# carolinebear/pytorch_end2end_speech_recognition

Measured on AMD Instinct MI355X. Metric: training frames/sec, higher is better.
Workload: dtype bf16; 1 GPU; librispeech100h_char_ctc_blstm5x512; batch_per_gpu=32, global_batch=32, max_frames=1000, feat_dim=80, vocab=29, parallelism=dp1

## Files before the change

### include/asr_hip.h

```cpp
#ifndef ASR_HIP_H_
#define ASR_HIP_H_

#include <stddef.h>
#include <stdint.h>

#ifdef __cplusplus
extern "C" {
#endif

#define ASR_OK 0
#define ASR_ERR_ARG (-1)
#define ASR_ERR_WORKSPACE (-2)
#define ASR_ERR_HIP (-3)
#define ASR_ERR_UNSUPPORTED (-4)

#define ASR_DT_F32 0
#define ASR_DT_BF16 1

const char* asr_version(void);
const char* asr_last_error(void);
int asr_arch_is_gfx950(void);

int asr_stream_create_cu_masked(int cu_begin, int cu_count, void** stream_out);
int asr_stream_destroy(void* stream);

size_t asr_ctc_workspace_bytes(int T, int B, int V, int max_label_len);
int asr_ctc_forward(const float* acts, long long stride_t, long long stride_b, int T, int B,
                    int V, const int32_t* labels_flat, const int32_t* label_lens,
                    const int32_t* act_lens, int max_label_len, int blank, int zero_infinity,
                    float* costs, float* loss_out, float loss_scale, void* workspace,
                    size_t ws_bytes, void* stream);
int asr_ctc_forward_lse(const float* acts, long long stride_t, long long stride_b, int T, int B,
                        int V, const float* lse_part, int nslab, const int32_t* labels_flat,
                        const int32_t* label_lens, const int32_t* act_lens, int max_label_len,
                        int blank, int zero_infinity, float* costs, float* loss_out,
                        float loss_scale, void* workspace, size_t ws_bytes, void* stream);
int asr_ctc_backward(const float* acts, long long stride_t, long long stride_b, int T, int B,
                     int V, const int32_t* labels_flat, const int32_t* label_lens,
                     const int32_t* act_lens, int max_label_len, int blank,
                     const float* grad_scale, float scale, float* grads, long long gstride_t,
                     long long gstride_b, const void* workspace, size_t ws_bytes, void* stream);
int asr_ctc_backward_bf16(const float* acts, long long stride_t, long long stride_b, int T, int B,
                          int V, const int32_t* labels_flat, const int32_t* label_lens,
                          const int32_t* act_lens, int max_label_len, int blank,
                          const float* grad_scale, float scale, uint16_t* grads,
                          long long gstride_t, long long gstride_b, int gld,
                          const void* workspace, size_t ws_bytes, void* stream);
size_t asr_ctc_bias_workspace_bytes(int T, int B, int V, int gld);
int asr_ctc_backward_bf16_db(const float* acts, long long stride_t, long long stride_b, int T,
                             int B, int V, const int32_t* labels_flat, const int32_t* label_lens,
                             const int32_t* act_lens, int max_label_len, int blank,
                             const float* grad_scale, float scale, uint16_t* grads,
                             long long gstride_t, long long gstride_b, int gld,
                             const void* workspace, size_t ws_bytes, float* dbias, void* bias_ws,
                             size_t bias_ws_bytes, void* stream);
int asr_ctc_fwd_bwd(const float* acts, long long stride_t, long long stride_b, int T, int B,
                    int V, const int32_t* labels_flat, const int32_t* label_lens,
                    const int32_t* act_lens, int max_label_len, int blank, int zero_infinity,
                    float* costs, float* grads, void* workspace, size_t ws_bytes, void* stream);

int asr_ctc_last_path(int* out2);
int asr_ctc_last_lattice_waves(void);
int asr_gemm_last_family(void);

typedef struct {
  long long stride_b;
  long long stride_t;
  int rows_per_b;
  int t_mul;
  int t_add;
  int t_limit;
  const int32_t* perm;
} asr_rowmap_t;

typedef struct {
  const void* ptr;
  int dtype;
  int trans;
  asr_rowmap_t map;
  long long bytes;
  int tap_group;
  int tap_pitch;
  int tap_sign;
} asr_operand_t;

typedef struct {
  asr_operand_t a;
  asr_operand_t b;
  float* c;
  asr_rowmap_t c_map;
  const float* bias;
  const float* bias2;
  int M, N, K;
  float alpha, beta;
  int batch;
  long long batch_stride_a, batch_stride_b, batch_stride_c;
  float drop_p;
  unsigned long long drop_seed;
  int c_dtype;
} asr_gemm_t;

typedef struct { int small_tiles, nosplit, n64_kmode; } asr_gemm_opts_t;

int asr_gemm(const asr_gemm_t* problems, int nprob, int compute_dtype, void* stream,
             const asr_gemm_opts_t* opts);

size_t asr_gemm_workspace_bytes(const asr_gemm_t* problems, int nprob,
                                const asr_gemm_opts_t* opts);
int asr_gemm_ws(const asr_gemm_t* problems, int nprob, int compute_dtype, void* workspace,
                size_t ws_bytes, void* stream, const asr_gemm_opts_t* opts);
int asr_gemm_lse_ws(const asr_gemm_t* problem, int compute_dtype, float* lse, void* workspace,
                    size_t ws_bytes, void* stream, const asr_gemm_opts_t* opts);

int asr_lstm_wgrad_gate(void* stream);

size_t asr_colsum_workspace_bytes(int M, int N);
int asr_colsum_accumulate(const float* g, long long ld, int M, int N, float alpha, float* out0,
                          float* out1, void* workspace, size_t ws_bytes, void* stream);
int asr_colsum_accumulate_bf16(const uint16_t* g, long long ld, int M, int N, float alpha,
                               float* out0, float* out1, void* workspace, size_t ws_bytes,
                               void* stream);

typedef struct {
  int ws_prezeroed, bwd_pin_kb, bwd_units;
  const int* dy_flags;
  int dy_c0, dy_epoch;
  unsigned long long* progress;
  int progress_q1, progress_q2;
} asr_lstm_opts_t;
size_t asr_lstm_workspace_bytes(int B, int H, int compute_dtype, int backward);
int asr_lstm_forward(float* gx_act, const void* whh_f, const void* whh_r, int w_dtype,
                     const int32_t* lens, int B, int T, int H, int compute_dtype, float* y,
                     float* cst, uint16_t* ybf, void* workspace, size_t ws_bytes, void* stream,
                     const asr_lstm_opts_t* opts);
int asr_lstm_backward(const float* dy, const void* whh_f, const void* whh_r, int w_dtype,
                      const int32_t* lens, int B, int T, int H, int compute_dtype, float* act_dg,
                      const float* cst, uint16_t* dgbf, void* workspace, size_t ws_bytes,
                      void* stream, const asr_lstm_opts_t* opts);
// ... 453 lines not shown
```

### pytorch_end2end_speech_recognition_amd/_native.py

```python
import ctypes
import os

import torch

_HERE = os.path.dirname(os.path.abspath(__file__))
LIB_PATH = os.environ.get('ASR_LIB_PATH') or os.path.join(_HERE, 'libasr_hip.so')

c_int = ctypes.c_int
c_ll = ctypes.c_longlong
c_float = ctypes.c_float
c_size = ctypes.c_size_t
c_vp = ctypes.c_void_p
c_str = ctypes.c_char_p

ASR_OK = 0
ASR_ERR_UNSUPPORTED = -4
ASR_DT_F32 = 0
ASR_DT_BF16 = 1

SIGNATURES = {
    'asr_version': (c_str, []),
    'asr_last_error': (c_str, []),
    'asr_arch_is_gfx950': (c_int, []),
    'asr_stream_create_cu_masked': (c_int, [c_int, c_int, c_vp]),
    'asr_stream_destroy': (c_int, [c_vp]),
    'asr_ctc_workspace_bytes': (c_size, [c_int, c_int, c_int, c_int]),
    'asr_ctc_forward': (c_int, [c_vp, c_ll, c_ll, c_int, c_int, c_int, c_vp, c_vp, c_vp, c_int,
                                c_int, c_int, c_vp, c_vp, c_float, c_vp, c_size, c_vp]),
    'asr_ctc_forward_lse': (c_int, [c_vp, c_ll, c_ll, c_int, c_int, c_int, c_vp, c_int, c_vp,
                                    c_vp, c_vp, c_int, c_int, c_int, c_vp, c_vp, c_float, c_vp,
                                    c_size, c_vp]),
    'asr_ctc_backward': (c_int, [c_vp, c_ll, c_ll, c_int, c_int, c_int, c_vp, c_vp, c_vp, c_int,
                                 c_int, c_vp, c_float, c_vp, c_ll, c_ll, c_vp, c_size, c_vp]),
    'asr_ctc_backward_bf16': (c_int, [c_vp, c_ll, c_ll, c_int, c_int, c_int, c_vp, c_vp, c_vp,
                                      c_int, c_int, c_vp, c_float, c_vp, c_ll, c_ll, c_int, c_vp,
                                      c_size, c_vp]),
    'asr_ctc_bias_workspace_bytes': (c_size, [c_int, c_int, c_int, c_int]),
    'asr_ctc_backward_bf16_db': (c_int, [c_vp, c_ll, c_ll, c_int, c_int, c_int, c_vp, c_vp, c_vp,
                                         c_int, c_int, c_vp, c_float, c_vp, c_ll, c_ll, c_int, c_vp,
                                         c_size, c_vp, c_vp, c_size, c_vp]),
    'asr_ctc_fwd_bwd': (c_int, [c_vp, c_ll, c_ll, c_int, c_int, c_int, c_vp, c_vp, c_vp, c_int,
                                c_int, c_int, c_vp, c_vp, c_vp, c_size, c_vp]),
    'asr_gemm': (c_int, [c_vp, c_int, c_int, c_vp, c_vp]),
    'asr_gemm_workspace_bytes': (c_size, [c_vp, c_int, c_vp]),
    'asr_gemm_ws': (c_int, [c_vp, c_int, c_int, c_vp, c_size, c_vp, c_vp]),
    'asr_gemm_lse_ws': (c_int, [c_vp, c_int, c_vp, c_vp, c_size, c_vp, c_vp]),
    'asr_lstm_wgrad_gate': (c_int, [c_vp]),
    'asr_colsum_workspace_bytes': (c_size, [c_int, c_int]),
    'asr_colsum_accumulate': (c_int, [c_vp, c_ll, c_int, c_int, c_float, c_vp, c_vp, c_vp, c_size,
                                      c_vp]),
    'asr_colsum_accumulate_bf16': (c_int, [c_vp, c_ll, c_int, c_int, c_float, c_vp, c_vp, c_vp,
                                           c_size, c_vp]),
    'asr_conv3x3_c1_forward_xs': (c_int, [c_vp, c_int, c_int, c_int, c_int, c_int, c_vp, c_vp,
                                          c_vp, c_int, c_vp]),
    'asr_conv3x3_tr_supported': (c_int, [c_int, c_int, c_int]),
    'asr_conv3x3_tr': (c_int, [c_vp, c_ll, c_int, c_int, c_int, c_vp, c_int, c_vp, c_vp, c_int,
                               c_vp]),
    'asr_vgg_zero_halo': (c_int, [c_vp, c_int, c_int, c_int, c_int, c_int, c_vp]),
    'asr_conv3x3_c1_wgrad_workspace_bytes': (c_size, [c_int]),
    'asr_conv3x3_c1_wgrad_xs': (c_int, [c_vp, c_int, c_int, c_int, c_int, c_int, c_vp, c_int, c_vp,
                                        c_vp, c_size, c_vp]),
    'asr_conv3x3_tr_wgrad_workspace_bytes': (c_size, [c_ll, c_int, c_int, c_int]),
    'asr_conv3x3_tr_wgrad': (c_int, [c_vp, c_vp, c_ll, c_int, c_int, c_int, c_vp, c_vp, c_size,
                                     c_vp]),
    'asr_conv3x3_c1_forward': (c_int, [c_vp, c_int, c_int, c_int, c_int, c_int, c_int, c_vp, c_vp,
                                       c_vp, c_vp]),
    'asr_lstm_workspace_bytes': (c_size, [c_int, c_int, c_int, c_int]),
    'asr_lstm_forward': (c_int, [c_vp, c_vp, c_vp, c_int, c_vp, c_int, c_int, c_int, c_int, c_vp,
                                 c_vp, c_vp, c_vp, c_size, c_vp, c_vp]),
    'asr_lstm_backward': (c_int, [c_vp, c_vp, c_vp, c_int, c_vp, c_int, c_int, c_int, c_int,
                                  c_vp, c_vp, c_vp, c_vp, c_size, c_vp, c_vp]),
    'asr_lstm_backward_db': (c_int, [c_vp, c_vp, c_vp, c_int, c_vp, c_int, c_int, c_int, c_int,
                                     c_vp, c_vp, c_vp, c_vp, c_vp, c_vp, c_size, c_vp, c_vp]),
    'asr_lstm_backward_dgbf': (c_int, [c_vp, c_vp, c_vp, c_int, c_vp, c_int, c_int, c_int, c_int,
                                       c_vp, c_vp, c_vp, c_vp, c_vp, c_vp, c_size, c_vp, c_vp]),
    'asr_lstm_forward_x': (c_int, [c_vp, c_int, c_vp, c_vp, c_vp, c_vp, c_vp, c_vp, c_int, c_int,
                                   c_int, c_vp, c_vp, c_vp, c_vp, c_vp, c_size, c_vp, c_vp]),
    'asr_lstm_forward_x_ok': (c_int, [c_int, c_int, c_int]),
    'asr_lstm_forward_xh': (c_int, [c_vp, c_int, c_vp, c_vp, c_vp, c_vp, c_vp, c_vp, c_int, c_int,
                                    c_int, c_vp, c_vp, c_vp, c_vp, c_vp, c_size, c_vp, c_vp]),
    'asr_lstm_forward_xh_drop': (c_int, [c_vp, c_int, c_vp, c_vp, c_vp, c_vp, c_vp, c_vp, c_int,
                                         c_int, c_int, c_vp, c_vp, c_vp, c_vp, c_vp, c_float,
                                         ctypes.c_ulonglong, c_vp, c_size, c_vp, c_vp]),
    'asr_lstm_backward_dgbf_h': (c_int, [c_vp, c_vp, c_vp, c_int, c_vp, c_int, c_int, c_int, c_int,
                                         c_vp, c_vp, c_vp, c_vp, c_vp, c_vp, c_size, c_vp, c_vp]),
    'asr_diag_lds_spin': (c_int, [c_int, c_int, c_vp, c_vp]),
    'asr_diag_hold_cus': (c_int, [c_int, c_int, c_int, c_vp]),
    'asr_lstm_unpack_act_h': (c_int, [c_vp, c_int, c_int, c_int, c_vp, c_vp]),
    'asr_gru_workspace_bytes': (c_size, [c_int, c_int]),
    'asr_gru_forward': (c_int, [c_vp, c_vp, c_vp, c_vp, c_int, c_int, c_int, c_vp, c_vp, c_vp]),
    'asr_gru_backward': (c_int, [c_vp, c_vp, c_vp, c_int, c_int, c_int, c_vp, c_vp, c_vp, c_vp,
                                 c_vp, c_size, c_vp]),
    'asr_gru_cell_forward': (c_int, [c_vp, c_vp, c_vp, c_int, c_int, c_vp, c_vp, c_vp]),
    'asr_gru_cell_backward': (c_int, [c_vp, c_vp, c_vp, c_vp, c_int, c_int, c_vp, c_vp, c_vp,
                                      c_vp]),
    'asr_grad_sqnorm_workspace_bytes': (c_size, []),
    'asr_grad_sqnorm': (c_int, [c_vp, c_ll, c_vp, c_vp, c_size, c_vp]),
    'asr_optim_step': (c_int, [c_int, c_vp, c_vp, c_vp, c_vp, c_ll, c_float, c_float, c_float,
                               c_float, c_float, c_ll, c_float, c_float, c_vp, c_float, c_vp,
                               c_vp]),
    'asr_optim_step_guarded': (c_int, [c_int, c_vp, c_vp, c_vp, c_vp, c_ll, c_float, c_float,
                                       c_float, c_float, c_float, c_ll, c_float, c_float, c_vp,
                                       c_float, c_vp, c_vp, c_vp]),
    'asr_dropout': (c_int, [c_vp, c_vp, c_ll, c_float, ctypes.c_ulonglong, c_vp]),
    'asr_embedding_forward': (c_int, [c_vp, c_vp, c_int, c_int, c_int, c_int, c_vp, c_vp]),
    'asr_embedding_backward': (c_int, [c_vp, c_vp, c_int, c_int, c_int, c_int, c_int, c_vp,
                                       c_vp]),
    'asr_embedding_backward_csr': (c_int, [c_vp, c_vp, c_vp, c_int, c_int, c_int, c_int, c_vp,
                                           c_vp]),
    'asr_tanh_forward': (c_int, [c_vp, c_vp, c_ll, c_vp]),
    'asr_tanh_backward': (c_int, [c_vp, c_vp, c_vp, c_ll, c_vp]),
    'asr_add_tanh_forward': (c_int, [c_vp, c_vp, c_vp, c_ll, c_vp]),
    'asr_add_forward': (c_int, [c_vp, c_vp, c_vp, c_ll, c_vp]),
    'asr_convert_rows_bf16': None,
    'asr_convert_rows_bf16_dropout': None,
    'asr_ctc_best_path': (c_int, [c_vp, c_ll, c_ll, c_int, c_int, c_int, c_vp, c_int, c_vp, c_vp,
                                  c_vp]),
    'asr_row_argmax': (c_int, [c_vp, c_int, c_int, c_vp, c_vp]),
    'asr_ctc_beam_ws_bytes': (c_size, [c_int, c_int, c_int, c_int]),
    'asr_ctc_beam_search': (c_int, [c_vp, c_ll, c_ll, c_int, c_int, c_int, c_vp, c_int, c_int,
                                    c_int, c_vp, c_size, c_vp, c_vp, c_vp, c_vp]),
    'asr_ctc_beam_rows': (c_int, [c_vp, c_ll, c_ll, c_int, c_int, c_int, c_vp, c_int, c_int, c_int,
                                  c_vp, c_size, c_vp]),
# ... 291 lines not shown
```

### pytorch_end2end_speech_recognition_amd/csrc/ctc.hip

```cpp
#include "common.h"
#include "prof.h"

namespace asr {
namespace {

constexpr int kMaxK = 16;

struct CtcWs {
  float* lse;
  float* emit;
  float* alpha;
  float* beta;
  float* logp;
  int32_t* offs;
  int32_t* status;
};

inline size_t align256(size_t x) { return (x + 255) & ~size_t(255); }

inline int pick_k(int max_label_len) {
  int S = 2 * max_label_len + 1;
  int k = 1;
  while (64 * k < S) k <<= 1;
  return k;
}

inline size_t ws_layout(int T, int B, int max_label_len, CtcWs* ws, char* base) {
  const int Spad = 64 * pick_k(max_label_len);
  size_t off = 0;
  auto take = [&](size_t bytes) { size_t o = off; off = align256(off + bytes); return base + o; };
  char* p;
  p = take(sizeof(float) * (size_t)B * T);                 if (ws) ws->lse = (float*)p;
  p = take(sizeof(float) * (size_t)B * T * Spad);          if (ws) ws->emit = (float*)p;
  p = take(sizeof(float) * (size_t)B * T * Spad);          if (ws) ws->alpha = (float*)p;
  p = take(sizeof(float) * (size_t)B * T * Spad);          if (ws) ws->beta = (float*)p;
  p = take(sizeof(float) * (size_t)B);                     if (ws) ws->logp = (float*)p;
  p = take(sizeof(int32_t) * (size_t)B);                   if (ws) ws->offs = (int32_t*)p;
  p = take(sizeof(int32_t) * 4);                           if (ws) ws->status = (int32_t*)p;
  return off;
}

__global__ void ctc_prep(const int32_t* __restrict__ label_lens, const int32_t* __restrict__ labels,
                         int B, int V, int blank, int max_label_len, int32_t* __restrict__ offs,
                         int32_t* __restrict__ status) {
  if (threadIdx.x == 0) {
    int acc = 0, bad = 0;
    for (int b = 0; b < B; ++b) {
      offs[b] = acc;
      int L = label_lens[b];
      if (L < 0 || L > max_label_len) bad |= 1;
      acc += L < 0 ? 0 : L;
    }
    status[0] = bad;
    status[1] = acc;
  }
  __syncthreads();
  int total = status[1];
  for (int i = threadIdx.x; i < total; i += blockDim.x) {
    int v = labels[i];
    if (v < 0 || v >= V || v == blank) atomicOr(&status[0], 2);
  }
}

__device__ __forceinline__ void lds_barrier() {
  asm volatile("s_waitcnt lgkmcnt(0)\n\ts_barrier" ::: "memory");
}

constexpr float kLog2e = 1.4426950408889634f;
constexpr float kLn2 = 0.6931471805599453f;
__device__ __forceinline__ float ex2(float x) { return __builtin_amdgcn_exp2f(x); }
__device__ __forceinline__ float lg2(float x) { return __builtin_amdgcn_logf(x); }

__device__ __forceinline__ void lse_acc4(float& m, float& s, float4 v) {
  const float mx = fmaxf(fmaxf(v.x, v.y), fmaxf(v.z, v.w));
  if (mx > m) { s *= __expf(m - mx); m = mx; }
  s += __expf(v.x - m) + __expf(v.y - m) + __expf(v.z - m) + __expf(v.w - m);
}
__device__ __forceinline__ void lse_acc1(float& m, float& s, float x) {
  if (x > m) { s *= __expf(m - x); m = x; }
  s += __expf(x - m);
}

__device__ __forceinline__ int head_elems(const float* p) {
// ... 982 lines not shown
  extern __shared__ __attribute__((aligned(16))) float lds_n[];
  const int lane = threadIdx.x & 63, wave = threadIdx.x >> 6;
  float* occ = lds_n + wave * V;
  const int n8 = gld >> 3;
  const float scale = (grad_scale ? grad_scale[0] : 1.0f) * scale_mul;
  float acc[NCH][8];
#pragma unroll
  for (int j = 0; j < NCH; ++j)
#pragma unroll
    for (int e = 0; e < 8; ++e) acc[j][e] = 0.f;
  for (int r = wave; r < rpb; r += NW) {
    const long long lin = (long long)blockIdx.x * rpb + r;
    if (lin >= nrows) break;
    const long long row = rev ? nrows - 1 - lin : lin;
    const int b = (int)(row / T), t = (int)(row % T);
    uint16_t* g = grads + (long long)t * gst + (long long)b * gsb;
    const float* x = acts + (long long)t * st + (long long)b * sb;
    const int Tb = act_lens[b];
    const float lp = logp[b];
    if (t >= Tb || lp == neg_inf()) {
      for (int i = lane; i < n8; i += 64) reinterpret_cast<uint4*>(g)[i] = make_uint4(0u, 0u, 0u, 0u);
      continue;
    }
    float xv[NCH][8];
#pragma unroll
    for (int j = 0; j < NCH; ++j)
#pragma unroll
      for (int e = 0; e < 8; ++e) {
        const int c = 8 * (lane + 64 * j) + e;
        xv[j][e] = c < V ? x[c] : 0.f;
      }
    const float z = lse[row];
    const int L = min(label_lens[b], (Spad - 1) / 2);
    const int S = 2 * L + 1;
    const int32_t* lab = labels + offs[b];
    const float* al = alpha + row * Spad;
    const float* bt = beta + row * Spad;
    const float* em = emit + row * Spad;
    for (int v = lane; v < V; v += 64) occ[v] = 0.f;
    __builtin_amdgcn_fence(__ATOMIC_RELEASE, "wavefront");
    __builtin_amdgcn_wave_barrier();
    for (int s_ = lane; s_ < S; s_ += 64) {
      int c = (s_ & 1) ? lab[s_ >> 1] : blank;
      c = c < 0 ? 0 : (c >= V ? V - 1 : c);
      atomicAdd(&occ[c], ex2(al[s_] + bt[s_] - em[s_] - lp));
    }
    __builtin_amdgcn_fence(__ATOMIC_ACQ_REL, "wavefront");
    __builtin_amdgcn_wave_barrier();
#pragma unroll
    for (int j = 0; j < NCH; ++j) {
      const int k = lane + 64 * j;
      if (k >= n8) continue;
      unsigned w[4];
#pragma unroll
      for (int q = 0; q < 4; ++q) {
        const int c = 8 * k + 2 * q;
        const float lo = c < V ? (__expf(xv[j][2 * q] - z) - occ[c]) * scale : 0.f;
        const float hi = c + 1 < V ? (__expf(xv[j][2 * q + 1] - z) - occ[c + 1]) * scale : 0.f;
        acc[j][2 * q] += lo;
        acc[j][2 * q + 1] += hi;
        w[q] = (c < V ? (unsigned)f2bf(lo) : 0u) | ((c + 1 < V ? (unsigned)f2bf(hi) : 0u) << 16);
      }
      reinterpret_cast<uint4*>(g)[k] = make_uint4(w[0], w[1], w[2], w[3]);
    }
    __builtin_amdgcn_fence(__ATOMIC_ACQ_REL, "wavefront");
    __builtin_amdgcn_wave_barrier();
  }
  if (!colpart) return;
  float* wp = lds_n + NW * V;
#pragma unroll
  for (int j = 0; j < NCH; ++j) {
    const int k = lane + 64 * j;
    if (k >= n8) continue;
#pragma unroll
    for (int e = 0; e < 8; ++e) wp[wave * gld + 8 * k + e] = acc[j][e];
  }
  __syncthreads();
  float* o = colpart + (long long)blockIdx.x * gld;
  for (int c = threadIdx.x; c < gld; c += 64 * NW) {
    float v = wp[c];
#pragma unroll
    for (int w = 1; w < NW; ++w) v += wp[w * gld + c];
    o[c] = v;
  }
}

template <int NCH>
__global__ void __launch_bounds__(256) ctc_grad_bf16_pipe(
    const float* __restrict__ acts, long long st, long long sb, int T, int V,
    const int32_t* __restrict__ labels, const int32_t* __restrict__ label_lens,
    const int32_t* __restrict__ act_lens, const int32_t* __restrict__ offs, int blank, int Spad,
    const float* __restrict__ lse, const float* __restrict__ emit,
    const float* __restrict__ alpha, const float* __restrict__ beta,
    const float* __restrict__ logp, const float* __restrict__ grad_scale, float scale_mul,
    uint16_t* __restrict__ grads, long long gst, long long gsb, int gld, int rev,
    int acts_bytes, float* __restrict__ colpart, int rpb, long long nrows) {
  extern __shared__ __attribute__((aligned(16))) float occ[];
  float* corr = occ + Spad;
  int* clsT = (int*)(occ + Spad + V);
  __shared__ int s_b;
  const int tid = threadIdx.x, nth = blockDim.x;
  const int n8 = gld >> 3;
  const float scale = (grad_scale ? grad_scale[0] : 1.0f) * scale_mul;
  const __amdgpu_buffer_rsrc_t rs =
      __builtin_amdgcn_make_buffer_rsrc((void*)acts, 0, acts_bytes, 0x00020000);
  float acc[NCH > 0 ? NCH : 1][8];
#pragma unroll
  for (int j = 0; j < (NCH > 0 ? NCH : 1); ++j)
#pragma unroll
    for (int e = 0; e < 8; ++e) acc[j][e] = 0.f;
  for (int v = tid; v < V; v += nth) corr[v] = 0.f;
  if (tid == 0) s_b = -1;
  struct Row { long long row; int b, t, Tb, L; float lp, z; float sv[4]; };
  auto fetch = [&](int r, Row& h) {
    const long long lin = (long long)blockIdx.x * rpb + r;
    h.row = rev ? nrows - 1 - lin : lin;
    h.b = (int)(h.row / T);
    h.t = (int)(h.row % T);
    h.Tb = act_lens[h.b];
    h.lp = logp[h.b];
    h.z = lse[h.row];
    h.L = label_lens[h.b];
    const long long so = h.row * Spad;
#pragma unroll
    for (int q = 0; q < 4; ++q) {
      const int s_ = tid + q * nth;
      h.sv[q] = s_ < Spad ? alpha[so + s_] + beta[so + s_] - emit[so + s_] : 0.f;
    }
  };
  const int nr = (int)min((long long)rpb, nrows - (long long)blockIdx.x * rpb);
  Row cur;
  if (nr > 0) fetch(0, cur);
  for (int r = 0; r < nr; ++r) {
    const int b = cur.b, t = cur.t;
    uint16_t* g = grads + (long long)t * gst + (long long)b * gsb;
    const bool live = t < cur.Tb && cur.lp != neg_inf();
    const int L = min(cur.L, (Spad - 1) / 2);
    const int S = 2 * L + 1;
    __syncthreads();
    if (live && s_b != b) {
      const int32_t* lab = labels + offs[b];
      for (int s_ = tid; s_ < S; s_ += nth) {
        int c = (s_ & 1) ? lab[s_ >> 1] : blank;
        clsT[s_] = c < 0 ? 0 : (c >= V ? V - 1 : c);
      }
    }
    if (live) {
#pragma unroll
      for (int q = 0; q < 4; ++q) {
        const int s_ = tid + q * nth;
        if (s_ < S) occ[s_] = ex2(cur.sv[q] - cur.lp);
      }
    }
    __syncthreads();
    if (tid == 0 && live) s_b = b;
    int rep_c[4] = {-1, -1, -1, -1};
    if (live) {
#pragma unroll
      for (int q4 = 0; q4 < 4; ++q4) {
        const int s_ = tid + q4 * nth;
        if (s_ >= S) continue;
        const int c = clsT[s_];
        bool first;
        if ((s_ & 1) == 0) {
          first = s_ == 0;
        } else {
// ... 606 lines not shown
#define ASR_CTC_GS(NC)                                                                           \
  hipLaunchKernelGGL((ctc_grad_bf16_stream<NC>), dim3((unsigned)nblk), dim3(512), lds2, s, acts, \
                     stride_t, stride_b, T, V, labels_flat, label_lens, act_lens, ws.offs, blank, \
                     Spad, ws.lse, ws.emit, ws.alpha, ws.beta, ws.logp, grad_scale, scale, grads, \
                     gstride_t, gstride_b, gld, rev, abytes, colpart, rpb, rows)
    switch (nchs) {
      case 1: ASR_CTC_GS(1); break;
      case 2: ASR_CTC_GS(2); break;
      default: ASR_CTC_GS(3); break;
    }
#undef ASR_CTC_GS
  } else
#define ASR_CTC_GP(NC)                                                                           \
  hipLaunchKernelGGL((ctc_grad_bf16_pipe<NC>), dim3((unsigned)nblk), dim3(threads), lds, s, acts, \
                     stride_t, stride_b, T, V, labels_flat, label_lens, act_lens, ws.offs, blank, \
                     Spad, ws.lse, ws.emit, ws.alpha, ws.beta, ws.logp, grad_scale, scale, grads, \
                     gstride_t, gstride_b, gld, rev, abytes, colpart, rpb, rows)
  if (pipe) {
    g_ctc_last_path[1] = 3;
    switch (nch) {
      case 1: ASR_CTC_GP(1); break;
      case 2: ASR_CTC_GP(2); break;
      case 4: ASR_CTC_GP(4); break;
      case 5: ASR_CTC_GP(5); break;
      default: ASR_CTC_GP(8); break;
    }
  } else if (table) {
    g_ctc_last_path[1] = 1;
    if (nch) ASR_CTC_G16A(true, 1, false);
    else ASR_CTC_G16A(true, 0, false);
  } else {
    g_ctc_last_path[1] = 1;
    switch (nch) {
      case 0: ASR_CTC_G16(false, 0); break;
      case 1: ASR_CTC_G16(false, 1); break;
      case 2: ASR_CTC_G16(false, 2); break;
      case 4: ASR_CTC_G16(false, 4); break;
      case 5: ASR_CTC_G16(false, 5); break;
      default: ASR_CTC_G16(false, 8); break;
    }
  }
#undef ASR_CTC_G16A
#undef ASR_CTC_GP
#undef ASR_CTC_G16
  ASR_LAUNCH_CHECK();
  prof_end_launch(ASR_PROF_CTC_GRAD, pslot, s);
  if (dbias) {
    const size_t part = ((size_t)nblk * gld * sizeof(float) + 255) & ~(size_t)255;
    rc = asr_colsum_accumulate(colpart, gld, nblk, V, 1.0f, dbias, nullptr, (char*)bws + part,
                               bws_bytes - part, stream);
    if (rc) return rc;
  }
  return ASR_OK;
}

extern "C" int asr_ctc_backward_bf16(const float* acts, long long stride_t, long long stride_b,
                                     int T, int B, int V, const int32_t* labels_flat,
                                     const int32_t* label_lens, const int32_t* act_lens,
                                     int max_label_len, int blank, const float* grad_scale,
                                     float scale, uint16_t* grads, long long gstride_t,
                                     long long gstride_b, int gld, const void* workspace,
                                     size_t ws_bytes, void* stream) {
  return ctc_backward_bf16_impl(acts, stride_t, stride_b, T, B, V, labels_flat, label_lens,
                                act_lens, max_label_len, blank, grad_scale, scale, grads,
                                gstride_t, gstride_b, gld, workspace, ws_bytes, nullptr, nullptr, 0,
                                stream);
}

extern "C" int asr_ctc_backward_bf16_db(const float* acts, long long stride_t, long long stride_b,
                                        int T, int B, int V, const int32_t* labels_flat,
                                        const int32_t* label_lens, const int32_t* act_lens,
                                        int max_label_len, int blank, const float* grad_scale,
                                        float scale, uint16_t* grads, long long gstride_t,
                                        long long gstride_b, int gld, const void* workspace,
                                        size_t ws_bytes, float* dbias, void* bias_ws,
                                        size_t bias_ws_bytes, void* stream) {
  ASR_REQUIRE(dbias, ASR_ERR_ARG, "ctc_bf16_db: dbias is null");
  return ctc_backward_bf16_impl(acts, stride_t, stride_b, T, B, V, labels_flat, label_lens,
                                act_lens, max_label_len, blank, grad_scale, scale, grads,
                                gstride_t, gstride_b, gld, workspace, ws_bytes, dbias, bias_ws,
                                bias_ws_bytes, stream);
}

extern "C" int asr_ctc_fwd_bwd(const float* acts, long long stride_t, long long stride_b, int T,
                               int B, int V, const int32_t* labels_flat,
                               const int32_t* label_lens, const int32_t* act_lens,
                               int max_label_len, int blank, int zero_infinity, float* costs,
                               float* grads, void* workspace, size_t ws_bytes, void* stream) {
  int rc = asr_ctc_forward(acts, stride_t, stride_b, T, B, V, labels_flat, label_lens, act_lens,
                           max_label_len, blank, zero_infinity, costs, nullptr, 1.f, workspace,
                           ws_bytes, stream);
  if (rc || !grads) return rc;
  return asr_ctc_backward(acts, stride_t, stride_b, T, B, V, labels_flat, label_lens, act_lens,
                          max_label_len, blank, nullptr, 1.f, grads, stride_t, stride_b, workspace,
                          ws_bytes, stream);
}
```

### pytorch_end2end_speech_recognition_amd/native_ops.py

```python
import collections
import ctypes
import os
import weakref

import numpy as np
import torch

from . import _native as N

F32 = N.ASR_DT_F32
BF16 = N.ASR_DT_BF16

_compute = {'dtype': F32}


def set_compute_dtype(name):
    if name not in ('fp32', 'bf16'):
        raise ValueError('compute dtype must be fp32 or bf16')
    _compute['dtype'] = BF16 if name == 'bf16' else F32


def compute_dtype():
    return _compute['dtype']

# ... 406 lines not shown
        ctx.beside = _beside_plan[0]
        return y

    @staticmethod
    def backward(ctx, dy):
        xo, wo = ctx.saved_tensors
        bias, stage, xshape, weight = ctx.meta
        dy = dy.contiguous()
        Nout = weight.shape[0]
        M = dy.numel() // Nout
        if M == 0:
            return torch.zeros(xshape, dtype=torch.float32, device=dy.device), None, None, None
        Np = wo.shape[0] if stage else Nout
        dyo = _staged(dy, M, Nout, Np) if stage else dy
        if ctx.beside is not None:
            dx = _linear_backward(xo, wo, bias, stage, xshape, weight, ctx.drop, dyo,
                                  ctx.needs_input_grad[0], dy_bias=dy, wgrad=False)
            gb = (grad_buffer(weight),) + ((grad_buffer(bias),) if bias is not None else ())
            wgrad = lambda go: _linear_wgrad(xo, wo, bias, stage, xshape, weight, dyo,
                                             dy_bias=dy, gemm_opts=go)
            if not _wgrad_beside(dy.device, ctx.beside, wgrad, (xo, wo, dyo, dy), gb):
                wgrad(None)
            return dx, None, None, None
        dx = _linear_backward(xo, wo, bias, stage, xshape, weight, ctx.drop, dyo,
                              ctx.needs_input_grad[0], dy_bias=dy)
        return dx, None, None, None


def _ctc_forward(logits, st, sb, T, B, V, lse, labels_flat, label_lens, act_lens, max_label_len,
                 blank, zero_infinity, costs, loss, loss_scale, ws, nbytes):
    common = (N.ptr(labels_flat), N.ptr(label_lens), N.ptr(act_lens), int(max_label_len),
              int(blank), int(bool(zero_infinity)), N.ptr(costs), N.ptr(loss), float(loss_scale),
              N.ptr(ws), nbytes, N.stream_handle(logits.device))
    if lse is not None:
        N.call('asr_ctc_forward_lse', N.ptr(logits), st, sb, T, B, V, N.ptr(lse), lse.shape[0],
               *common)
    else:
        N.call('asr_ctc_forward', N.ptr(logits), st, sb, T, B, V, *common)


class LinearCTCFn(torch.autograd.Function):

    @staticmethod
    def forward(ctx, x, weight, bias, drop, labels_flat, label_lens, act_lens, max_label_len,
                loss_scale, blank, zero_infinity):
        N.require_device(labels_flat, label_lens, act_lens)
        V = weight.shape[0]
        M = x.numel() // x.shape[-1]
        lse = (torch.empty((V + 63) // 64, M, 2, dtype=torch.float32, device=x.device)
               if _ctc_lse_epilogue(V) and M > 0 else None)
        logits, xo, wo, stage = _linear_forward(x, weight, bias, drop, lse=lse,
                                                ld=(V + 3) // 4 * 4 if V > 1024 else V)
        assert stage, 'LinearCTCFn needs a staged (bf16) output layer'
        B, T, V = logits.shape
        nbytes = N.query('asr_ctc_workspace_bytes', T, B, V, max_label_len)
        ws = _ws(nbytes, logits.device)
        costs = torch.empty(B, dtype=torch.float32, device=logits.device)
        loss = torch.empty(1, dtype=torch.float32, device=logits.device)
        _ctc_forward(logits, logits.stride(1), logits.stride(0), T, B, V, lse, labels_flat,
                     label_lens, act_lens, max_label_len, blank, zero_infinity, costs, loss,
                     loss_scale, ws, nbytes)
        ctx.save_for_backward(xo, wo, logits, labels_flat, label_lens, act_lens, ws)
        ctx.meta = (bias, tuple(x.shape), weight, int(max_label_len), int(blank),
                    float(loss_scale), nbytes)
        ctx.from_blstm = _produced_by_blstm(x)
        ctx.drop = drop
        ctx.mark_non_differentiable(costs)
        return loss, costs

    @staticmethod
    def backward(ctx, g_loss, g_costs):
        xo, wo, logits, labels_flat, label_lens, act_lens, ws = ctx.saved_tensors
        bias, xshape, weight, max_label_len, blank, loss_scale, nbytes = ctx.meta
        B, T, V = logits.shape
        Np = wo.shape[0]
        dev = logits.device
        dyo = torch.empty(B * T, Np, dtype=torch.bfloat16, device=dev)
        g = g_loss.contiguous() if g_loss is not None else None
        args = (N.ptr(logits), logits.stride(1), logits.stride(0), T, B, V, N.ptr(labels_flat),
                N.ptr(label_lens),
                N.ptr(act_lens), max_label_len, blank, N.ptr(g),
                loss_scale if g is not None else 0.0, N.ptr(dyo), Np, T * Np, Np, N.ptr(ws), nbytes)
        bws = None
        if bias is not None and V <= 16384 and os.environ.get('ASR_CTC_HEAD_DB', '1') != '0':
            bnb = N.query('asr_ctc_bias_workspace_bytes', T, B, V, Np)
            bws = _ws(bnb, dev)
            N.call('asr_ctc_backward_bf16_db', *args, N.ptr(grad_buffer(bias)), N.ptr(bws), bnb,
                   N.stream_handle(dev))
        else:
            N.call('asr_ctc_backward_bf16', *args, N.stream_handle(dev))
        bias_w = None if bws is not None else bias
        if ctx.from_blstm is not None and os.environ.get('ASR_HEAD_WGRAD_SIDE', '1') != '0':
            dx = _linear_backward(xo, wo, bias_w, True, xshape, weight, ctx.drop, dyo,
                                  ctx.needs_input_grad[0], dy_bias=dyo, wgrad=False)
            gb = (grad_buffer(weight),) + ((grad_buffer(bias),) if bias is not None else ())
            wgrad = lambda go: _linear_wgrad(xo, wo, bias_w, True, xshape, weight, dyo,
                                             dy_bias=dyo, gemm_opts=go)
            if not _wgrad_beside(dev, ctx.from_blstm, wgrad, (xo, wo, dyo), gb):
                wgrad(None)
            return (dx,) + (None,) * 10
        dx = _linear_backward(xo, wo, bias_w, True, xshape, weight, ctx.drop, dyo,
                              ctx.needs_input_grad[0], dy_bias=dyo)
        return (dx,) + (None,) * 10


class LinearCTC32Fn(torch.autograd.Function):

    @staticmethod
    def forward(ctx, x, weight, bias, drop, labels_flat, label_lens, act_lens, max_label_len,
                loss_scale, blank, zero_infinity):
        N.require_device(x, weight, labels_flat, label_lens, act_lens)
        ctx.from_blstm = _produced_by_blstm(x)
        x = x.contiguous()
        B, T, K = x.shape
        V = weight.shape[0]
        Vp = (V + 3) // 4 * 4
        dev = x.device
        if drop is not None:
            xd = torch.empty_like(x)
            N.call('asr_dropout', N.ptr(x), N.ptr(xd), x.numel(), float(drop[0]), int(drop[1]),
                   N.stream_handle(dev))
            x = xd
        logits = torch.empty(B * T, Vp, dtype=torch.float32, device=dev)
        lse = (torch.empty((V + 63) // 64, B * T, 2, dtype=torch.float32, device=dev)
               if _ctc_lse_epilogue(V) and B * T > 0 else None)
        if B * T > 0:
            run_gemm([gemm_problem(operand(x, 0, rowmap(K)), operand(weight, 0, rowmap(K)),
                                   logits, rowmap(Vp), B * T, V, K, bias=bias)], dev, lse=lse)
        nbytes = N.query('asr_ctc_workspace_bytes', T, B, V, max_label_len)
        ws = _ws(nbytes, dev)
        costs = torch.empty(B, dtype=torch.float32, device=dev)
        loss = torch.empty(1, dtype=torch.float32, device=dev)
        _ctc_forward(logits, Vp, T * Vp, T, B, V, lse, labels_flat, label_lens, act_lens,
                     max_label_len, blank, zero_infinity, costs, loss, loss_scale, ws, nbytes)
        ctx.save_for_backward(x, logits, labels_flat, label_lens, act_lens, ws)
        ctx.meta = (bias, weight, B, T, V, Vp, int(max_label_len), int(blank), float(loss_scale),
                    nbytes)
        ctx.drop = drop
        ctx.mark_non_differentiable(costs)
        return loss, costs

    @staticmethod
    def backward(ctx, g_loss, g_costs):
        x, logits, labels_flat, label_lens, act_lens, ws = ctx.saved_tensors
        bias, weight, B, T, V, Vp, max_label_len, blank, loss_scale, nbytes = ctx.meta
        dev = logits.device
        K = x.shape[-1]
        M = B * T
        dl = torch.empty(M, Vp, dtype=torch.float32, device=dev)
        g = g_loss.contiguous() if g_loss is not None else None
        N.call('asr_ctc_backward', N.ptr(logits), Vp, T * Vp, T, B, V, N.ptr(labels_flat),
               N.ptr(label_lens), N.ptr(act_lens), max_label_len, blank, N.ptr(g),
               loss_scale if g is not None else 0.0, N.ptr(dl), Vp, T * Vp, N.ptr(ws), nbytes,
               N.stream_handle(dev))
        dx = None
        if ctx.needs_input_grad[0]:
            dx = torch.empty(B, T, K, dtype=torch.float32, device=dev)
            if M > 0:
                run_gemm([gemm_problem(operand(dl, 0, rowmap(Vp)), operand(weight, 1, rowmap(K)),
                                       dx, rowmap(K), M, K, V, drop=ctx.drop)], dev)

        def wgrad(gemm_opts):
            if M > 0:
                run_gemm([gemm_problem(operand(dl, 1, rowmap(Vp)), operand(x, 1, rowmap(K)),
                                       grad_buffer(weight), rowmap(K), V, K, M, beta=1.0)], dev,
                         opts=gemm_opts)
            if bias is not None:
                colsum_accumulate(dl[:, :V], grad_buffer(bias))
        gb = (grad_buffer(weight),) + ((grad_buffer(bias),) if bias is not None else ())
        if not (ctx.from_blstm is not None and os.environ.get('ASR_HEAD_WGRAD_SIDE', '1') != '0'
                and _wgrad_beside(dev, ctx.from_blstm, wgrad, (x, dl), gb)):
            wgrad(None)
        return (dx,) + (None,) * 10


def _produced_by_blstm(t, depth=4):
    frontier = [t.grad_fn] if t.grad_fn is not None else []
    for _ in range(depth):
        nxt = []
        for fn in frontier:
            if fn is None:
                continue
            if type(fn).__name__.startswith('BLSTMLayerFn'):
                return getattr(fn, 'bh', None)
            nxt.extend(f for f, _ in getattr(fn, 'next_functions', ()))
        frontier = nxt
# ... 2365 lines not shown
```

Baseline: 1.760 million frames/s.

## Fuse CTC head gradient with output-projection dgrad GEMM via MFMA

Adds a CTC backward kernel that computes the bf16 logit gradients and, in the same pass, multiplies each 16-row tile by the projection weight with MFMA to produce the input gradient (with dropout applied) directly. The Python autograd path uses it when V<=256 and the shapes fit, and skips the separate dx GEMM. This removes a separate GEMM launch and a re-read of the logit-gradient buffer. In exchange, weights are held in registers, LDS use grows, and the dx GEMM now runs on a narrow 16-row tile that may use MFMA less efficiently than a tuned GEMM.

```diff
diff --git a/include/asr_hip.h b/include/asr_hip.h
--- a/include/asr_hip.h
+++ b/include/asr_hip.h
@@ -54,6 +54,15 @@
                              long long gstride_t, long long gstride_b, int gld,
                              const void* workspace, size_t ws_bytes, float* dbias, void* bias_ws,
                              size_t bias_ws_bytes, void* stream);
+int asr_ctc_backward_bf16_dx_ok(int T, int B, int V, int gld, int K);
+int asr_ctc_backward_bf16_dx(const float* acts, long long stride_t, long long stride_b, int T,
+                             int B, int V, const int32_t* labels_flat, const int32_t* label_lens,
+                             const int32_t* act_lens, int max_label_len, int blank,
+                             const float* grad_scale, float scale, uint16_t* grads,
+                             long long gstride_t, long long gstride_b, int gld,
+                             const void* workspace, size_t ws_bytes, float* dbias, void* bias_ws,
+                             size_t bias_ws_bytes, int fuse_dx, const uint16_t* wo, int K,
+                             float* dx, float drop_p, unsigned long long drop_seed, void* stream);
 int asr_ctc_fwd_bwd(const float* acts, long long stride_t, long long stride_b, int T, int B,
                     int V, const int32_t* labels_flat, const int32_t* label_lens,
                     const int32_t* act_lens, int max_label_len, int blank, int zero_infinity,
diff --git a/pytorch_end2end_speech_recognition_amd/_native.py b/pytorch_end2end_speech_recognition_amd/_native.py
--- a/pytorch_end2end_speech_recognition_amd/_native.py
+++ b/pytorch_end2end_speech_recognition_amd/_native.py
@@ -39,6 +39,11 @@
     'asr_ctc_backward_bf16_db': (c_int, [c_vp, c_ll, c_ll, c_int, c_int, c_int, c_vp, c_vp, c_vp,
                                          c_int, c_int, c_vp, c_float, c_vp, c_ll, c_ll, c_int, c_vp,
                                          c_size, c_vp, c_vp, c_size, c_vp]),
+    'asr_ctc_backward_bf16_dx_ok': (c_int, [c_int, c_int, c_int, c_int, c_int]),
+    'asr_ctc_backward_bf16_dx': (c_int, [c_vp, c_ll, c_ll, c_int, c_int, c_int, c_vp, c_vp, c_vp,
+                                         c_int, c_int, c_vp, c_float, c_vp, c_ll, c_ll, c_int, c_vp,
+                                         c_size, c_vp, c_vp, c_size, c_int, c_vp, c_int, c_vp,
+                                         c_float, ctypes.c_ulonglong, c_vp]),
     'asr_ctc_fwd_bwd': (c_int, [c_vp, c_ll, c_ll, c_int, c_int, c_int, c_vp, c_vp, c_vp, c_int,
                                 c_int, c_int, c_vp, c_vp, c_vp, c_size, c_vp]),
     'asr_gemm': (c_int, [c_vp, c_int, c_int, c_vp, c_vp]),
diff --git a/pytorch_end2end_speech_recognition_amd/csrc/ctc.hip b/pytorch_end2end_speech_recognition_amd/csrc/ctc.hip
--- a/pytorch_end2end_speech_recognition_amd/csrc/ctc.hip
+++ b/pytorch_end2end_speech_recognition_amd/csrc/ctc.hip
@@ -1,4 +1,5 @@
 #include "common.h"
+#include "mfma.h"
 #include "prof.h"
 
 namespace asr {
@@ -1147,6 +1148,159 @@
 #pragma unroll
     for (int w = 1; w < NW; ++w) v += wp[w * gld + c];
     o[c] = v;
+  }
+}
+
+template <int TPW, int KS>
+__global__ void __launch_bounds__(512) ctc_grad_dx_narrow(
+    const float* __restrict__ acts, long long st, long long sb, int T, int V,
+    const int32_t* __restrict__ labels, const int32_t* __restrict__ label_lens,
+    const int32_t* __restrict__ act_lens, const int32_t* __restrict__ offs, int blank, int Spad,
+    const float* __restrict__ lse, const float* __restrict__ emit,
+    const float* __restrict__ alpha, const float* __restrict__ beta,
+    const float* __restrict__ logp, const float* __restrict__ grad_scale, float scale_mul,
+    uint16_t* __restrict__ grads, long long gst, long long gsb, int gld, int rev,
+    float* __restrict__ colpart, int rpb, int nsub, long long nblk, long long nrows,
+    const uint16_t* __restrict__ wo, int K, float* __restrict__ dx, float drop_p,
+    unsigned long long drop_seed) {
+  constexpr int NW = 8;
+  extern __shared__ __attribute__((aligned(16))) float lds_x[];
+  const int lane = threadIdx.x & 63;
+  const int wave = __builtin_amdgcn_readfirstlane(threadIdx.x >> 6);
+  float* occ = lds_x + wave * V;
+  float* rowval = lds_x + NW * V;
+  const int apitch = gld + 8;
+  uint16_t* atile = reinterpret_cast<uint16_t*>(rowval + (colpart ? 2 * 16 * gld : 0));
+  const int n8 = gld >> 3;
+  const int RW = nsub * rpb;
+  const long long nruns = (nrows + RW - 1) / RW;
+  const float scale = (grad_scale ? grad_scale[0] : 1.0f) * scale_mul;
+  const int lm = lane & 15, lg = lane >> 4;
+
+  bf16x8 fw[TPW][KS];
+#pragma unroll
+  for (int t = 0; t < TPW; ++t) {
+    const int n = (wave * TPW + t) * 16 + lm;
+#pragma unroll
+    for (int ks = 0; ks < KS; ++ks) {
+      u16x8 v = u16x8{0, 0, 0, 0, 0, 0, 0, 0};
+#pragma unroll
+      for (int j = 0; j < 8; ++j) {
+        const int k = 32 * ks + 8 * lg + j;
+        if (n < K && k < gld) v[j] = wo[(long long)k * K + n];
+      }
+      fw[t][ks] = as_bf16x8(v);
+    }
+  }
+
+  int it = 0;
+  for (long long run = blockIdx.x; run < nruns; run += gridDim.x, ++it) {
+    float* rv = rowval + (it & 1) * 16 * gld;
+    uint16_t* at = atile + (it & 1) * 16 * apitch;
+    for (int r = wave; r < 16; r += NW) {
+      const long long lin = run * RW + r;
+      uint4* arow = reinterpret_cast<uint4*>(at + r * apitch);
+      float* rvrow = rv + r * gld;
+      const bool inside = r < RW && lin < nrows;
+      const long long row = rev ? nrows - 1 - lin : lin;
+      const int b = inside ? (int)(row / T) : 0, t = inside ? (int)(row % T) : 0;
+      uint16_t* g = grads + (long long)t * gst + (long long)b * gsb;
+      const float* x = acts + (long long)t * st + (long long)b * sb;
+      const int Tb = act_lens[b];
+      const float lp = logp[b];
+      if (!inside || t >= Tb || lp == neg_inf()) {
+        if (lane < n8) {
+          arow[lane] = make_uint4(0u, 0u, 0u, 0u);
+          if (inside) reinterpret_cast<uint4*>(g)[lane] = make_uint4(0u, 0u, 0u, 0u);
+          if (colpart) {
+            *reinterpret_cast<f32x4*>(rvrow + 8 * lane) = f32x4{0.f, 0.f, 0.f, 0.f};
+            *reinterpret_cast<f32x4*>(rvrow + 8 * lane + 4) = f32x4{0.f, 0.f, 0.f, 0.f};
+          }
+        }
+        continue;
+      }
+      float xv[8];
+#pragma unroll
+      for (int e = 0; e < 8; ++e) {
+        const int c = 8 * lane + e;
+        xv[e] = c < V ? x[c] : 0.f;
+      }
+      const float z = lse[row];
+      const int L = min(label_lens[b], (Spad - 1) / 2);
+      const int S = 2 * L + 1;
+      const int32_t* lab = labels + offs[b];
+      const float* al = alpha + row * Spad;
+      const float* bt = beta + row * Spad;
+      const float* em = emit + row * Spad;
+      for (int v = lane; v < V; v += 64) occ[v] = 0.f;
+      __builtin_amdgcn_fence(__ATOMIC_RELEASE, "wavefront");
+      __builtin_amdgcn_wave_barrier();
+      for (int s_ = lane; s_ < S; s_ += 64) {
+        int c = (s_ & 1) ? lab[s_ >> 1] : blank;
+        c = c < 0 ? 0 : (c >= V ? V - 1 : c);
+        atomicAdd(&occ[c], ex2(al[s_] + bt[s_] - em[s_] - lp));
+      }
+      __builtin_amdgcn_fence(__ATOMIC_ACQ_REL, "wavefront");
+      __builtin_amdgcn_wave_barrier();
+      if (lane < n8) {
+        unsigned w[4];
+        float f[8];
+#pragma unroll
+        for (int q = 0; q < 4; ++q) {
+          const int c = 8 * lane + 2 * q;
+          const float lo = c < V ? (__expf(xv[2 * q] - z) - occ[c]) * scale : 0.f;
+          const float hi = c + 1 < V ? (__expf(xv[2 * q + 1] - z) - occ[c + 1]) * scale : 0.f;
+          f[2 * q] = 0.f + lo;
+          f[2 * q + 1] = 0.f + hi;
+          w[q] = (c < V ? (unsigned)f2bf(lo) : 0u) | ((c + 1 < V ? (unsigned)f2bf(hi) : 0u) << 16);
+        }
+        const uint4 w4 = make_uint4(w[0], w[1], w[2], w[3]);
+        reinterpret_cast<uint4*>(g)[lane] = w4;
+        arow[lane] = w4;
+        if (colpart) {
+          *reinterpret_cast<f32x4*>(rvrow + 8 * lane) = f32x4{f[0], f[1], f[2], f[3]};
+          *reinterpret_cast<f32x4*>(rvrow + 8 * lane + 4) = f32x4{f[4], f[5], f[6], f[7]};
+        }
+      }
+      __builtin_amdgcn_fence(__ATOMIC_ACQ_REL, "wavefront");
+      __builtin_amdgcn_wave_barrier();
+    }
+    __syncthreads();
+    if (colpart) {
+      for (int i = threadIdx.x; i < nsub * gld; i += 64 * NW) {
+        const int k = i / gld, c = i - k * gld;
+        const long long blk = run * nsub + k;
+        if (blk >= nblk) continue;
+        const float* p = rv + (k * rpb) * gld + c;
+        float v = p[0];
+        for (int j = 1; j < rpb; ++j) v += p[j * gld];
+        colpart[blk * gld + c] = v;
+      }
+    }
+    bf16x8 fa[KS];
+#pragma unroll
+    for (int ks = 0; ks < KS; ++ks) {
+      const int k = 32 * ks + 8 * lg;
+      fa[ks] = k < gld ? load_bf16x8(at + lm * apitch + k) : as_bf16x8(u16x8{0, 0, 0, 0, 0, 0, 0, 0});
+    }
+    const long long lin = run * RW + lm;
+    const bool rok = lm < RW && lin < nrows;
+    const long long row = rev ? nrows - 1 - lin : lin;
+#pragma unroll
+    for (int t = 0; t < TPW; ++t) {
+      const int n0 = (wave * TPW + t) * 16;
+      if (n0 >= K) break;
+      f32x4 acc = f32x4{0.f, 0.f, 0.f, 0.f};
+#pragma unroll
+      for (int ks = 0; ks < KS; ++ks)
+        if (32 * ks < gld) acc = mfma_bf16(fw[t][ks], fa[ks], acc);
+      const int n = n0 + 4 * lg;
+      if (!rok || n >= K) continue;
+      const long long off = row * K + n;
+      float o[4] = {acc[0], acc[1], acc[2], acc[3]};
+      if (drop_p > 0.f) drop_n<4>(o, drop_p, drop_seed, (unsigned long long)off);
+      *reinterpret_cast<f32x4*>(dx + off) = f32x4{o[0], o[1], o[2], o[3]};
+    }
   }
 }
 
@@ -1919,6 +2073,118 @@
                                 bias_ws_bytes, stream);
 }
 
+static bool ctc_dx_tiles(int gld, int K, int* tpw, int* ks) {
+  if (gld < 8 || gld > 256 || gld % 8 || K < 8 || K % 8) return false;
+  auto pow2 = [](int v) { int p = 1; while (p < v) p <<= 1; return p; };
+  *tpw = pow2(((K + 15) / 16 + 7) / 8);
+  *ks = pow2((gld + 31) / 32);
+  return *tpw * *ks <= 8;
+}
+
+extern "C" int asr_ctc_backward_bf16_dx_ok(int T, int B, int V, int gld, int K) {
+  int tpw, ks, rpb, nblk;
+  if (T <= 0 || B <= 0 || V <= 1 || V > 256 || gld < V || !ctc_dx_tiles(gld, K, &tpw, &ks))
+    return 0;
+  ctc_bias_grid(T, B, V, &rpb, &nblk);
+  return rpb <= 4;
+}
+
+extern "C" int asr_ctc_backward_bf16_dx(const float* acts, long long stride_t, long long stride_b,
+                                        int T, int B, int V, const int32_t* labels_flat,
+                                        const int32_t* label_lens, const int32_t* act_lens,
+                                        int max_label_len, int blank, const float* grad_scale,
+                                        float scale, uint16_t* grads, long long gstride_t,
+                                        long long gstride_b, int gld, const void* workspace,
+                                        size_t ws_bytes, float* dbias, void* bias_ws,
+                                        size_t bias_ws_bytes, int fuse_dx, const uint16_t* wo,
+                                        int K, float* dx, float drop_p,
+                                        unsigned long long drop_seed, void* stream) {
+  if (!fuse_dx)
+    return ctc_backward_bf16_impl(acts, stride_t, stride_b, T, B, V, labels_flat, label_lens,
+                                  act_lens, max_label_len, blank, grad_scale, scale, grads,
+                                  gstride_t, gstride_b, gld, workspace, ws_bytes, dbias,
+                                  dbias ? bias_ws : nullptr, dbias ? bias_ws_bytes : 0, stream);
+  int rc = check_common(acts, T, B, V, labels_flat, label_lens, act_lens, max_label_len, blank,
+                        workspace, ws_bytes);
+  if (rc) return rc;
+  ASR_REQUIRE(grads && wo && dx, ASR_ERR_ARG, "ctc_bf16_dx: null pointer argument");
+  ASR_REQUIRE(gld >= V && gld % 8 == 0 && gstride_t % 8 == 0 && gstride_b % 8 == 0 &&
+                  ((uintptr_t)grads & 15) == 0 && ((uintptr_t)dx & 15) == 0,
+              ASR_ERR_ARG, "ctc_bf16_dx: gradient rows must be 16-B aligned with gld %d >= V %d",
+              gld, V);
+  ASR_REQUIRE(drop_p >= 0.f && drop_p < 1.f, ASR_ERR_ARG, "ctc_bf16_dx: dropout p outside [0, 1)");
+  int tpw = 0, ks = 0;
+  ASR_REQUIRE(asr_ctc_backward_bf16_dx_ok(T, B, V, gld, K) && ctc_dx_tiles(gld, K, &tpw, &ks),
+              ASR_ERR_UNSUPPORTED,
+              "ctc_bf16_dx: V %d, gld %d, K %d is outside the fused kernel's limits "
+              "(asr_ctc_backward_bf16_dx_ok)", V, gld, K);
+  hipStream_t s = (hipStream_t)stream;
+  CtcWs ws;
+  ws_layout(T, B, max_label_len, &ws, (char*)workspace);
+  const int Spad = 64 * pick_k(max_label_len);
+  const long long rows = (long long)B * T;
+  const int rev = (ctc_row_order() >> 1) & 1;
+  int rpb = 4, nblk = (int)((rows + 3) / 4);
+  float* colpart = nullptr;
+  if (dbias) {
+    ASR_REQUIRE(bias_ws && bias_ws_bytes >= asr_ctc_bias_workspace_bytes(T, B, V, gld),
+                ASR_ERR_WORKSPACE, "ctc_bf16_dx: bias workspace %zu < %zu", bias_ws_bytes,
+                asr_ctc_bias_workspace_bytes(T, B, V, gld));
+    ctc_bias_grid(T, B, V, &rpb, &nblk);
+    colpart = (float*)bias_ws;
+  }
+  const int nsub = 16 / rpb;
+  const long long nruns = (rows + nsub * rpb - 1) / (nsub * rpb);
+  const size_t lds = (size_t)(8 * V + (dbias ? 2 * 16 * gld : 0)) * sizeof(float) +
+                     (size_t)2 * 16 * (gld + 8) * sizeof(uint16_t);
+  static int cus = 0;
+  if (cus == 0) {
+    int dev = 0;
+    if (hipGetDevice(&dev) != hipSuccess ||
+        hipDeviceGetAttribute(&cus, hipDeviceAttributeMultiprocessorCount, dev) != hipSuccess ||
+        cus <= 0)
+      cus = 256;
+  }
+  const int pslot = prof_begin_launch(ASR_PROF_CTC_GRAD, s,
+                                      (4.0 * V + 2.0 * gld + 4.0 * K) * (double)rows, V);
+  g_ctc_last_path[1] = 5;
+#define ASR_CTC_DX(TP, KSS)                                                                      \
+  static int occ##TP##KSS = 0;                                                                   \
+  if (occ##TP##KSS == 0 &&                                                                       \
+      (hipOccupancyMaxActiveBlocksPerMultiprocessor(&occ##TP##KSS, ctc_grad_dx_narrow<TP, KSS>,  \
+                                                    512, 48 * 1024) != hipSuccess ||             \
+       occ##TP##KSS < 1))                                                                        \
+    occ##TP##KSS = 1;                                                                            \
+  const int grid = (int)std::min<long long>(nruns, (long long)occ##TP##KSS * cus);               \
+  hipLaunchKernelGGL((ctc_grad_dx_narrow<TP, KSS>), dim3((unsigned)grid), dim3(512), lds, s,     \
+                     acts, stride_t, stride_b, T, V, labels_flat, label_lens, act_lens, ws.offs, \
+                     blank, Spad, ws.lse, ws.emit, ws.alpha, ws.beta, ws.logp, grad_scale,       \
+                     scale, grads, gstride_t, gstride_b, gld, rev, colpart, rpb, nsub,           \
+                     (long long)nblk, rows, wo, K, dx, drop_p, drop_seed)
+  switch (tpw * 16 + ks) {
+    case 1 * 16 + 1: { ASR_CTC_DX(1, 1); break; }
+    case 1 * 16 + 2: { ASR_CTC_DX(1, 2); break; }
+    case 1 * 16 + 4: { ASR_CTC_DX(1, 4); break; }
+    case 1 * 16 + 8: { ASR_CTC_DX(1, 8); break; }
+    case 2 * 16 + 1: { ASR_CTC_DX(2, 1); break; }
+    case 2 * 16 + 2: { ASR_CTC_DX(2, 2); break; }
+    case 2 * 16 + 4: { ASR_CTC_DX(2, 4); break; }
+    case 4 * 16 + 1: { ASR_CTC_DX(4, 1); break; }
+    case 4 * 16 + 2: { ASR_CTC_DX(4, 2); break; }
+    default: { ASR_CTC_DX(8, 1); break; }
+  }
+#undef ASR_CTC_DX
+  ASR_LAUNCH_CHECK();
+  prof_end_launch(ASR_PROF_CTC_GRAD, pslot, s);
+  if (dbias) {
+    const size_t part = ((size_t)nblk * gld * sizeof(float) + 255) & ~(size_t)255;
+    rc = asr_colsum_accumulate(colpart, gld, nblk, V, 1.0f, dbias, nullptr,
+                               (char*)bias_ws + part, bias_ws_bytes - part, stream);
+    if (rc) return rc;
+  }
+  return ASR_OK;
+}
+
 extern "C" int asr_ctc_fwd_bwd(const float* acts, long long stride_t, long long stride_b, int T,
                                int B, int V, const int32_t* labels_flat,
                                const int32_t* label_lens, const int32_t* act_lens,
diff --git a/pytorch_end2end_speech_recognition_amd/native_ops.py b/pytorch_end2end_speech_recognition_amd/native_ops.py
--- a/pytorch_end2end_speech_recognition_amd/native_ops.py
+++ b/pytorch_end2end_speech_recognition_amd/native_ops.py
@@ -512,9 +512,26 @@
                 N.ptr(act_lens), max_label_len, blank, N.ptr(g),
                 loss_scale if g is not None else 0.0, N.ptr(dyo), Np, T * Np, Np, N.ptr(ws), nbytes)
         bws = None
+        bnb = 0
         if bias is not None and V <= 16384 and os.environ.get('ASR_CTC_HEAD_DB', '1') != '0':
             bnb = N.query('asr_ctc_bias_workspace_bytes', T, B, V, Np)
             bws = _ws(bnb, dev)
+        need_dx = ctx.needs_input_grad[0]
+        K = xshape[-1]
+        fuse_dx = (need_dx and V <= 256 and K % 8 == 0 and wo.shape[1] == K and
+                   os.environ.get('ASR_CTC_HEAD_DX_FUSED', '1') != '0' and
+                   hasattr(N.lib(), 'asr_ctc_backward_bf16_dx') and
+                   N.query('asr_ctc_backward_bf16_dx_ok', T, B, V, Np, K) == 1)
+        dx_fused = None
+        if fuse_dx:
+            dx_fused = torch.empty(xshape, dtype=torch.float32, device=dev)
+            drop = ctx.drop
+            N.call('asr_ctc_backward_bf16_dx', *args,
+                   N.ptr(grad_buffer(bias)) if bws is not None else None, N.ptr(bws), bnb, 1,
+                   N.ptr(wo), K, N.ptr(dx_fused), float(drop[0]) if drop else 0.0,
+                   int(drop[1]) if drop else 0, N.stream_handle(dev))
+            need_dx = False
+        elif bws is not None:
             N.call('asr_ctc_backward_bf16_db', *args, N.ptr(grad_buffer(bias)), N.ptr(bws), bnb,
                    N.stream_handle(dev))
         else:
@@ -522,16 +539,16 @@
         bias_w = None if bws is not None else bias
         if ctx.from_blstm is not None and os.environ.get('ASR_HEAD_WGRAD_SIDE', '1') != '0':
             dx = _linear_backward(xo, wo, bias_w, True, xshape, weight, ctx.drop, dyo,
-                                  ctx.needs_input_grad[0], dy_bias=dyo, wgrad=False)
+                                  need_dx, dy_bias=dyo, wgrad=False)
             gb = (grad_buffer(weight),) + ((grad_buffer(bias),) if bias is not None else ())
             wgrad = lambda go: _linear_wgrad(xo, wo, bias_w, True, xshape, weight, dyo,
                                              dy_bias=dyo, gemm_opts=go)
             if not _wgrad_beside(dev, ctx.from_blstm, wgrad, (xo, wo, dyo), gb):
                 wgrad(None)
-            return (dx,) + (None,) * 10
+            return (dx_fused if fuse_dx else dx,) + (None,) * 10
         dx = _linear_backward(xo, wo, bias_w, True, xshape, weight, ctx.drop, dyo,
-                              ctx.needs_input_grad[0], dy_bias=dyo)
-        return (dx,) + (None,) * 10
+                              need_dx, dy_bias=dyo)
+        return (dx_fused if fuse_dx else dx,) + (None,) * 10
 
 
 class LinearCTC32Fn(torch.autograd.Function):
```

Result: no change. 1.762 million frames/s, median of 6 (+0.2%).
